# ku222/Attention-GAN

Hardware: AMD Instinct MI355X
Metric: train images/sec at 256×256 stage-3, batch 24/GPU, 1/2/4/8 MI355X (higher is better)
Workload: dtype f32; 1 GPU; full 3-stage AttnGAN 64->128->256 train step: G + 3xD updates + word attention + DAMSM words/sentence loss + KL + 4x fused Adam (BASELINE.json configs[2]); workload_key=full3, batch_per_gpu=24, global_batch=24, gf_dim=32, df_dim=64, emb_dim=256, seq_len=10, text_encoder=bypassed (frozen; N(0,1) embeddings), parallelism=dp1, discriminator_streams=3, launch=eager, gradient_exchange=none (one rank), losses_finite=True

## Files before the change

attention-gan_amd/csrc/conv_wino.hip:

```cpp
#include "conv_common.h"

#include <cstring>

using namespace agan;
using namespace agan::conv;

namespace {

typedef unsigned u32x4 __attribute__((ext_vector_type(4)));

__device__ __forceinline__ void lds_barrier_w() { asm volatile("s_waitcnt lgkmcnt(0)\n\ts_barrier" ::: "memory"); }

__global__ __launch_bounds__(256) void wino_weight_transform_kernel(const float* __restrict__ wk, float* __restrict__ U, int Kin, int Nld, int N) {
    const int total = Kin * Nld;
    for (int e = blockIdx.x * 256 + threadIdx.x; e < total; e += gridDim.x * 256) {
        const int n = e % Nld, c = e / Nld;
        float gk[3][3];
#pragma unroll
        for (int r = 0; r < 3; ++r)
#pragma unroll
            for (int s = 0; s < 3; ++s) gk[r][s] = n < N ? wk[(size_t)(c * 9 + r * 3 + s) * Nld + n] : 0.f;
        float t[4][3];
#pragma unroll
        for (int s = 0; s < 3; ++s) {
            t[0][s] = gk[0][s];
            t[1][s] = 0.5f * (gk[0][s] + gk[1][s] + gk[2][s]);
            t[2][s] = 0.5f * (gk[0][s] - gk[1][s] + gk[2][s]);
            t[3][s] = gk[2][s];
        }
        const int nch8 = Kin >> 3;
#pragma unroll
        for (int xi = 0; xi < 4; ++xi) {
            const float u0 = t[xi][0], u1 = 0.5f * (t[xi][0] + t[xi][1] + t[xi][2]), u2 = 0.5f * (t[xi][0] - t[xi][1] + t[xi][2]), u3 = t[xi][2];
            const float u[4] = {u0, u1, u2, u3};
#pragma unroll
            for (int nu = 0; nu < 4; ++nu) U[((size_t)((xi * 4 + nu) * nch8 + (c >> 3)) * Nld + n) * 8 + (c & 7)] = u[nu];
        }
    }
}

struct WinoTraits {
    int step, extra, origin;
    int cch;
    int planes, classes;
    int stages, nacc;
    int vfrags;
    int pieces;
    int ni32, ni64;
    int lds_cap;
    int s_u_second, s_raw_load, s_u_next, s_transform, s_raw_store;
    bool mulshift;
    bool store1_late;
};
constexpr WinoTraits wino_traits(WinoKind k) {
    WinoTraits t{};
    t.origin = -1; t.classes = 1; t.lds_cap = 160 * 1024; t.s_u_second = 0; t.s_raw_load = 1;
    switch (k) {
    case WinoKind::conv3x3:
        t.step = 2; t.extra = 2; t.cch = 8; t.planes = 16; t.stages = 16; t.nacc = 16; t.vfrags = 16; t.pieces = 4; t.ni32 = 7; t.ni64 = 11;
        t.s_u_next = 8; t.s_transform = 1; t.s_raw_store = 14;
        break;
    case WinoKind::conv3x3_half:
        t.step = 2; t.extra = 2; t.cch = 8; t.planes = 16; t.stages = 8; t.nacc = 8; t.vfrags = 16; t.pieces = 4; t.ni32 = 7;
        t.s_u_next = 4; t.s_transform = 1; t.s_raw_store = 6; t.lds_cap = 80 * 1024; t.mulshift = true;
        break;
    case WinoKind::conv4x4_s2:
        t.step = 4; t.extra = 2; t.cch = 8; t.planes = 36; t.stages = 36; t.nacc = 9; t.vfrags = 36; t.pieces = 4; t.ni32 = 21;
        t.s_u_next = 18; t.s_transform = 2; t.s_raw_store = 32; t.store1_late = true;
        break;
    case WinoKind::dgrad2x2_class:
        t.step = 2; t.extra = 1; t.cch = 16; t.planes = 36; t.classes = 4; t.stages = 18; t.nacc = 9; t.vfrags = 18; t.pieces = 2; t.ni32 = 11;
        t.s_u_next = 9; t.s_transform = 2; t.s_raw_store = 15; t.store1_late = true;
        break;
    }
    return t;
}

template <int D>
__device__ __forceinline__ void wino_input_f22(const float* src, int pcp, float* o, int pp) {
    float t[3][3];
#pragma unroll
    for (int j = 0; j < 3; ++j) {
        const float d0 = src[D * j], d1 = src[D * pcp + D * j], d2 = src[2 * D * pcp + D * j];
        t[0][j] = d0 - d1; t[1][j] = d1; t[2][j] = d2 - d1;
    }
#pragma unroll
    for (int xi = 0; xi < 3; ++xi) {
        o[(xi * 3 + 0) * pp] = t[xi][0] - t[xi][1]; o[(xi * 3 + 1) * pp] = t[xi][1]; o[(xi * 3 + 2) * pp] = t[xi][2] - t[xi][1];
    }
}

template <int NACC>
__device__ __forceinline__ void wino_output_2x2(const f32x16 (&acc)[NACC], int r, float (&y)[4]) {
    if constexpr (NACC == 16) {
        float c0[4], c1[4];
#pragma unroll
        for (int nu = 0; nu < 4; ++nu) {
            c0[nu] = acc[0 + nu][r] + acc[4 + nu][r] + acc[8 + nu][r];
            c1[nu] = acc[4 + nu][r] - acc[8 + nu][r] - acc[12 + nu][r];
        }
        y[0] = c0[0] + c0[1] + c0[2]; y[1] = c0[1] - c0[2] - c0[3];
        y[2] = c1[0] + c1[1] + c1[2]; y[3] = c1[1] - c1[2] - c1[3];
    } else {
        static_assert(NACC == 9, "F(2x2, 3x3) or F(2x2, 2x2)");
        float c0[3], c1[3];
#pragma unroll
        for (int nu = 0; nu < 3; ++nu) {
            c0[nu] = acc[nu][r] + acc[3 + nu][r];
            c1[nu] = acc[3 + nu][r] + acc[6 + nu][r];
        }
        y[0] = c0[0] + c0[1]; y[1] = c0[1] + c0[2];
        y[2] = c1[0] + c1[1]; y[3] = c1[1] + c1[2];
    }
}

template <WinoKind K, int NTG>
struct WinoGather {
    static constexpr WinoTraits T = wino_traits(K);
    static constexpr bool kHalf = K == WinoKind::conv3x3_half, kS2 = K == WinoKind::conv4x4_s2, kCls = K == WinoKind::dgrad2x2_class;
    static constexpr bool k3x3 = T.nacc != 9;
    static constexpr int NFW = kHalf ? 2 : 4 / NTG;
    static constexpr int NTL = 32 * NTG, LT = NTG == 1 ? 5 : 6;
    static constexpr int NI = NTG == 1 ? T.ni32 : T.ni64;
    static constexpr int CCH = T.cch, C8 = T.cch / 8;
    static constexpr int S = T.stages, SH = T.stages / 2, NACC = T.nacc;
    static constexpr int NPIECE = T.pieces * NTG;
    static constexpr int VBUF = T.vfrags * NTL * 8;
    static constexpr int STEP = T.step;
    static_assert(NI > 0, "this block size of the variant is not built: plan_wino must not route to it");
    static_assert(T.s_u_next == SH && T.s_transform + NPIECE <= S && T.s_raw_store < S, "slots of the chunk loop");

    const Geom& g;
    const WinoPlan& wp;
    int tid, lane, w, fw, tg, hh, l31, lh;
    int mt, nt, ks, py, px;
    int n0, txl, tyl, TX, TY, tx0, ty0, tb0, ihw, ohw, PR, PC, PCP, RAWBUF;
    float *raw, *V;
    __amdgpu_buffer_rsrc_t rx, rU;
    int nch8, c_beg, nch;
    int iy0, ix0;

    __device__ __forceinline__ WinoGather(const float* x, const float* U, const Geom& g_, const WinoPlan& wp_) : g(g_), wp(wp_) {
        extern __shared__ __attribute__((aligned(16))) unsigned char lds[];
        tid = threadIdx.x; lane = tid & 63;
        w = __builtin_amdgcn_readfirstlane(tid >> 6);
        fw = w % NFW; tg = kHalf ? 0 : w / NFW; hh = kHalf ? w / NFW : 0;
        l31 = lane & 31; lh = lane >> 5;
        ks = py = px = 0;
        {
            int F = xcd_contiguous(linear_block_id(), wp.mtiles * wp.ntiles * (kS2 ? wp.ksplit : T.classes));
            nt = F % wp.ntiles; F /= wp.ntiles;
            if constexpr (kS2) { mt = F % wp.mtiles; ks = F / wp.mtiles; }
            else if constexpr (kCls) { py = (F & 3) >> 1; px = F & 1; mt = F >> 2; }
            else mt = F;
        }
        n0 = nt * (NFW * 32);
        txl = wp.txl; tyl = wp.tyl;
        TX = 1 << txl; TY = 1 << tyl;
        const int bxi = mt % wp.blocks_x, byi = (mt / wp.blocks_x) % wp.blocks_y, bbi = mt / (wp.blocks_x * wp.blocks_y);
        tx0 = bxi << txl; ty0 = byi << tyl; tb0 = bbi << (LT - txl - tyl);
        ihw = g.IH * g.IW; ohw = g.OH * g.OW;
        PR = STEP * TY + T.extra; PC = STEP * TX + T.extra;
        PCP = wp.pcp;
        raw = reinterpret_cast<float*>(lds);
        RAWBUF = wp.raw_bytes >> 2;
        V = reinterpret_cast<float*>(lds + 2 * wp.raw_bytes);
        nch8 = g.Cin >> 3;
        if constexpr (kS2) { c_beg = ks * wp.chunks_per_split; nch = min(nch8, c_beg + wp.chunks_per_split) - c_beg; }
        else { c_beg = 0; nch = g.Cin >> (CCH == 8 ? 3 : 4); }
        constexpr int PPC = T.planes / T.classes;
        rx = make_rsrc(x, (size_t)g.B * g.Cin * ihw * sizeof(float));
        rU = make_rsrc(U + (size_t)(py * 2 + px) * PPC * nch8 * g.Nld * 8, (size_t)PPC * nch8 * g.Nld * 8 * sizeof(float));
        iy0 = STEP * ty0 + T.origin + py; ix0 = STEP * tx0 + T.origin + px;
    }

    __device__ __forceinline__ void stage_items(int (&it_off)[NI], unsigned (&it_lds)[NI]) const {
#pragma unroll
        for (int i = 0; i < NI; ++i) {
            const int e = tid + i * 256;
            int col, row, t2;
            if constexpr (T.mulshift) {
                const int t1 = (int)(__umul24(e, wp.mpc) >> 16);
                col = e - (int)__umul24(t1, PC);
                t2 = (int)(__umul24(t1, wp.mpr) >> 16); row = t1 - (int)__umul24(t2, PR);
            } else {
                col = e % PC; const int t1 = e / PC;
                row = t1 % PR; t2 = t1 / PR;
            }
            const int ci = t2 & (CCH - 1), b = tb0 + (t2 >> (CCH == 8 ? 3 : 4)), iy = iy0 + row, ix = ix0 + col;
            const bool ok = (e < wp.raw_items) & (b < g.B) & ((unsigned)iy < (unsigned)g.IH) & ((unsigned)ix < (unsigned)g.IW);
            if constexpr (T.mulshift) {
                it_off[i] = ok ? (int)__umul24(b * g.Cin + ci, ihw) + iy * g.IW + ix : -1;
                it_lds[i] = (unsigned)((int)__umul24(__umul24(t2, PR) + row, PCP) + col);
            } else {
                it_off[i] = ok ? (b * g.Cin + ci) * ihw + iy * g.IW + ix : -1;
                it_lds[i] = (unsigned)((t2 * PR + row) * PCP + col);
            }
        }
    }

    __device__ __forceinline__ void load_raw(const int (&it_off)[NI], int ch, float (&rv)[NI]) const {
#pragma unroll
        for (int i = 0; i < NI; ++i)
            rv[i] = buf_load_s(rx, it_off[i] >= 0 ? (unsigned)it_off[i] * 4u : kOOB, (unsigned)((c_beg + ch) * CCH * ihw) * 4u);
    }
    __device__ __forceinline__ void store_raw(const unsigned (&it_lds)[NI], int ch, const float (&rv)[NI]) const {
        float* const rb = raw + (ch & 1) * RAWBUF;
#pragma unroll
        for (int i = 0; i < NI; ++i)
            if (tid + i * 256 < wp.raw_items) rb[it_lds[i]] = rv[i];
    }
    __device__ __forceinline__ void load_u(int ch, int half, u32x4 (&uf)[SH]) const {
        const unsigned ulane = (unsigned)(min(n0 + fw * 32 + l31, g.Nld - 1) * 32 + lh * 16);
#pragma unroll
        for (int q = 0; q < SH; ++q) {
            const int s = half * SH + q;
            uf[q] = __builtin_bit_cast(u32x4, __builtin_amdgcn_raw_buffer_load_b128(
                rU, ulane, (unsigned)(((hh * S + s / C8) * nch8 + (c_beg + min(ch, nch - 1)) * C8 + s % C8) * g.Nld) * 32u, 0));
        }
    }

    __device__ __forceinline__ void transform_piece(const float* rb, float* Vb, int pi, float (&td)[NTG][4][4]) const {
        const int k = pi / T.pieces, sub = pi % T.pieces;
        const int tt = (tid >> 3) + 32 * k, ci = (tid & 7) + (kCls ? 8 * sub : 0);
        const int p = kS2 ? sub >> 1 : 0, q = kS2 ? sub & 1 : 0;
        if (!k3x3 || sub == 0) {
            const int ttx = tt & (TX - 1), tty = (tt >> txl) & (TY - 1), ttb = tt >> (txl + tyl);
            const float* const src = rb + ((ttb * CCH + ci) * PR + STEP * tty + p) * PCP + STEP * ttx + q;
            if constexpr (k3x3) {
                float d[4][4];
#pragma unroll
                for (int i = 0; i < 4; ++i) {
                    const float2 a = *reinterpret_cast<const float2*>(src + i * PCP), b = *reinterpret_cast<const float2*>(src + i * PCP + 2);
                    d[i][0] = a.x; d[i][1] = a.y; d[i][2] = b.x; d[i][3] = b.y;
                }
#pragma unroll
                for (int j = 0; j < 4; ++j) {
                    td[k][0][j] = d[0][j] - d[2][j];
                    td[k][1][j] = d[1][j] + d[2][j];
                    td[k][2][j] = d[2][j] - d[1][j];
                    td[k][3][j] = d[1][j] - d[3][j];
                }
            } else if constexpr (kS2) wino_input_f22<2>(src, PCP, Vb + (sub * 9 * NTL + tt) * 8 + ci, NTL * 8);
            else wino_input_f22<1>(src, PCP, Vb + tt * 16 + ci, NTL * 16);
        }
        if constexpr (k3x3) {
            const float (&t)[4] = td[k][sub];
            float* const o = Vb + (sub * 4 * NTL + tt) * 8 + ci;
            o[0] = t[0] - t[2]; o[NTL * 8] = t[1] + t[2]; o[2 * NTL * 8] = t[2] - t[1]; o[3 * NTL * 8] = t[1] - t[3];
        }
    }

    __device__ __forceinline__ void accumulate(f32x16 (&acc)[NACC]) const {
        int it_off[NI];
        unsigned it_lds[NI];
        stage_items(it_off, it_lds);
        float rawv[NI];
        float td[NTG][4][4];
        u32x4 ua[SH], ub[SH];
#pragma unroll
        for (int q = 0; q < NACC; ++q)
#pragma unroll
            for (int r = 0; r < 16; ++r) acc[q][r] = 0.f;
        {
            float rawv1[NI];
            load_raw(it_off, 0, rawv);
            if (!T.store1_late && nch > 1) load_raw(it_off, 1, rawv1);
            load_u(0, 0, ua);
            store_raw(it_lds, 0, rawv);
            if (nch > 1) {
                if constexpr (T.store1_late) load_raw(it_off, 1, rawv);
                else store_raw(it_lds, 1, rawv1);
            }
            lds_barrier_w();
#pragma unroll
            for (int pi = 0; pi < NPIECE; ++pi) transform_piece(raw, V, pi, td);
            if (T.store1_late && nch > 1) store_raw(it_lds, 1, rawv);
            lds_barrier_w();
        }
#pragma unroll 1
        for (int ch = 0; ch < nch; ++ch) {
            const float* Vc = V + (ch & 1) * VBUF;
            float* Vn = V + ((ch + 1) & 1) * VBUF;
            const float* rn = raw + ((ch + 1) & 1) * RAWBUF;
            const bool more = ch + 1 < nch;
            const unsigned vlane = (unsigned)(hh * S * NTL * 8 + (tg * 32 + l31) * CCH + lh * 4);
            u32x4 vf[2];
            vf[0] = *reinterpret_cast<const u32x4*>(Vc + vlane);
#pragma unroll
            for (int st = 0; st < S; ++st) {
                if (st + 1 < S) vf[(st + 1) & 1] = *reinterpret_cast<const u32x4*>(Vc + ((st + 1) / C8) * NTL * CCH + ((st + 1) % C8) * 8 + vlane);
                if (st == T.s_u_second) load_u(ch, 1, ub);
                if (st == T.s_raw_load && ch + 2 < nch) load_raw(it_off, ch + 2, rawv);
                if (st == T.s_u_next) load_u(ch + 1, 0, ua);
                if (more && st >= T.s_transform && st < T.s_transform + NPIECE) transform_piece(rn, Vn, st - T.s_transform, td);
                if (st == T.s_raw_store && ch + 2 < nch) store_raw(it_lds, ch + 2, rawv);
                const u32x4 uf = st < SH ? ua[st % SH] : ub[st % SH];
                const int a = kS2 ? st % NACC : st / C8;
#pragma unroll
                for (int j = 0; j < 4; ++j)
                    acc[a] = __builtin_amdgcn_mfma_f32_32x32x2f32(__uint_as_float(uf[j]), __uint_as_float(vf[st & 1][j]), acc[a], 0, 0, 0);
                __builtin_amdgcn_sched_barrier(0);
            }
            lds_barrier_w();
        }
    }

    __device__ __forceinline__ void epilogue(const f32x16 (&acc)[NACC], float* out) const {
        typedef float f32x2_ __attribute__((ext_vector_type(2)));
        typedef unsigned u32x2_ __attribute__((ext_vector_type(2)));
        const int lt = tg * 32 + l31;
        const int tx = lt & (TX - 1), ty = (lt >> txl) & (TY - 1), tb = lt >> (txl + tyl);
        const int b = tb0 + tb, oy = 2 * (ty0 + ty), ox = 2 * (tx0 + tx);
        const bool pvalid = (b < g.B) & (oy < (kCls ? g.OHs : g.OH)) & (ox < (kCls ? g.OWs : g.OW));
        const __amdgpu_buffer_rsrc_t ro = make_rsrc(out + (size_t)ks * wp.slab, (size_t)g.B * g.Cout * ohw * sizeof(float));
        const int nw = n0 + fw * 32;
#pragma unroll
        for (int r = 0; r < 16; ++r) {
            float y[4];
            wino_output_2x2(acc, r, y);
            const int n = nw + (r & 3) + 8 * (r >> 2) + 4 * lh;
            const bool ok = pvalid & (n < g.Cout);
            if constexpr (kCls) {
                const unsigned off = (unsigned)((b * g.Cout + n) * ohw + (2 * oy + py) * g.OW + 2 * ox + px) * 4u;
                buf_store(ro, ok ? off : kOOB, y[0]);
                buf_store(ro, ok ? off + 8u : kOOB, y[1]);
                buf_store(ro, ok ? off + (unsigned)(2 * g.OW) * 4u : kOOB, y[2]);
                buf_store(ro, ok ? off + (unsigned)(2 * g.OW + 2) * 4u : kOOB, y[3]);
            } else {
                const unsigned off = (unsigned)((b * g.Cout + n) * ohw + oy * g.OW + ox) * 4u;
                __builtin_amdgcn_raw_buffer_store_b64(__builtin_bit_cast(u32x2_, f32x2_{y[0], y[1]}), ro, ok ? off : kOOB, 0, 0);
                __builtin_amdgcn_raw_buffer_store_b64(__builtin_bit_cast(u32x2_, f32x2_{y[2], y[3]}), ro, ok ? off + (unsigned)g.OW * 4u : kOOB, 0, 0);
            }
        }
    }
};

template <int NFW>
__global__ __launch_bounds__(256, 1) void conv_wino_f32_kernel(const float* __restrict__ x, const float* __restrict__ U, float* __restrict__ out,
                                                               const Geom g, const WinoPlan wp) {
    WinoGather<WinoKind::conv3x3, 4 / NFW> k(x, U, g, wp);
    f32x16 acc[k.NACC];
    k.accumulate(acc);
    k.epilogue(acc, out);
}

__global__ __launch_bounds__(256, 2) void conv_wino_h_f32_kernel(const float* __restrict__ x, const float* __restrict__ U, float* __restrict__ out,
                                                                 const Geom g, const WinoPlan wp) {
    WinoGather<WinoKind::conv3x3_half, 1> k(x, U, g, wp);
    f32x16 acc[8];
    k.accumulate(acc);

    const int w = k.w, lane = k.lane, hh = k.hh, ohw = k.ohw;
    float* const X = k.raw;
    typedef float f32x2_ __attribute__((ext_vector_type(2)));
    typedef unsigned u32x2_ __attribute__((ext_vector_type(2)));
    const int tx = k.l31 & (k.TX - 1), ty = (k.l31 >> k.txl) & (k.TY - 1), tb = k.l31 >> (k.txl + k.tyl);
    const int b = k.tb0 + tb, oy = 2 * (k.ty0 + ty) + hh, ox = 2 * (k.tx0 + tx);
    const bool pvalid = (b < g.B) & (oy < g.OH) & (ox < g.OW);
    const __amdgpu_buffer_rsrc_t ro = make_rsrc(out, (size_t)g.B * g.Cout * ohw * sizeof(float));
    const int nw = k.n0 + k.fw * 32, pw = w ^ 2;
    const unsigned vo = pvalid ? (unsigned)((b * g.Cout + nw + 4 * k.lh) * ohw + oy * g.OW + ox) * 4u : kOOB;
    auto finish = [&](auto hc) {
        constexpr int HH = decltype(hc)::value;
        f32x2_ keep[8][2];
#pragma unroll
        for (int rp = 0; rp < 8; ++rp) {
            f32x2_ t[2][2];
#pragma unroll
            for (int x2 = 0; x2 < 2; ++x2) {
                const f32x2_ m0 = {acc[x2 * 4 + 0][2 * rp], acc[x2 * 4 + 0][2 * rp + 1]};
                const f32x2_ m1 = {acc[x2 * 4 + 1][2 * rp], acc[x2 * 4 + 1][2 * rp + 1]};
                const f32x2_ m2 = {acc[x2 * 4 + 2][2 * rp], acc[x2 * 4 + 2][2 * rp + 1]};
                const f32x2_ m3 = {acc[x2 * 4 + 3][2 * rp], acc[x2 * 4 + 3][2 * rp + 1]};
                t[x2][0] = m0 + m1 + m2;
                t[x2][1] = m1 - m2 - m3;
            }
#pragma unroll
            for (int c = 0; c < 2; ++c) {
                keep[rp][c] = t[0][c] + t[1][c];
                const f32x2_ send = HH == 0 ? t[1][c] : t[0][c];
                X[(w * 32 + (2 * rp) * 2 + c) * 64 + lane] = send[0];
                X[(w * 32 + (2 * rp + 1) * 2 + c) * 64 + lane] = send[1];
            }
        }
        lds_barrier_w();
#pragma unroll
        for (int r = 0; r < 16; ++r) {
            if (nw + 8 * (r >> 2) < g.Cout) {
                const float x0 = X[(pw * 32 + r * 2 + 0) * 64 + lane], x1 = X[(pw * 32 + r * 2 + 1) * 64 + lane];
                const float k0 = keep[r >> 1][0][r & 1], k1 = keep[r >> 1][1][r & 1];
                const f32x2_ y = HH == 0 ? f32x2_{x0 + k0, x1 + k1} : f32x2_{x0 - k0, x1 - k1};
                __builtin_amdgcn_raw_buffer_store_b64(__builtin_bit_cast(u32x2_, y), ro, vo, (unsigned)(((r & 3) + 8 * (r >> 2)) * ohw) * 4u, 0);
            }
        }
    };
    if (hh == 0) finish(std::integral_constant<int, 0>{});
    else finish(std::integral_constant<int, 1>{});
}

template <int NFW>
__global__ __launch_bounds__(256, 1) void conv_wino_s2_f32_kernel(const float* __restrict__ x, const float* __restrict__ U, float* __restrict__ out,
                                                                  const Geom g, const WinoPlan wp) {
    WinoGather<WinoKind::conv4x4_s2, 4 / NFW> k(x, U, g, wp);
    f32x16 acc[k.NACC];
    k.accumulate(acc);
    k.epilogue(acc, out);
}

template <int NFW>
__global__ __launch_bounds__(256, 1) void conv_wino_cls_f32_kernel(const float* __restrict__ x, const float* __restrict__ U, float* __restrict__ out,
                                                                   const Geom g, const WinoPlan wp) {
    WinoGather<WinoKind::dgrad2x2_class, 4 / NFW> k(x, U, g, wp);
    f32x16 acc[k.NACC];
    k.accumulate(acc);
    k.epilogue(acc, out);
}

__device__ __forceinline__ void wino_weights_f22(const float (&gk)[2][2], float* o, size_t pp) {
    const float t[3][2] = {{gk[0][0], gk[0][1]}, {gk[0][0] + gk[1][0], gk[0][1] + gk[1][1]}, {gk[1][0], gk[1][1]}};
#pragma unroll
    for (int xi = 0; xi < 3; ++xi) {
        const float u[3] = {t[xi][0], t[xi][0] + t[xi][1], t[xi][1]};
#pragma unroll
        for (int nu = 0; nu < 3; ++nu) o[(xi * 3 + nu) * pp] = u[nu];
    }
}

__global__ __launch_bounds__(256) void wino_cls_weight_transform_kernel(const float* __restrict__ wk, float* __restrict__ U, int Kin, int Nld, int N) {
    const int total = 4 * Kin * Nld, nch8 = Kin >> 3;
    for (int e = blockIdx.x * 256 + threadIdx.x; e < total; e += gridDim.x * 256) {
        const int n = e % Nld, t1 = e / Nld, c = t1 % Kin, cls = t1 / Kin;
        const float* wc = wk + (size_t)cls * Kin * 4 * Nld;
        float gk[2][2];
#pragma unroll
        for (int a = 0; a < 2; ++a)
#pragma unroll
            for (int b = 0; b < 2; ++b) gk[a][b] = n < N ? wc[(size_t)(c * 4 + (1 - a) * 2 + (1 - b)) * Nld + n] : 0.f;
        wino_weights_f22(gk, U + ((size_t)(cls * 9 * nch8 + (c >> 3)) * Nld + n) * 8 + (c & 7), (size_t)nch8 * Nld * 8);
    }
}

__global__ __launch_bounds__(256) void wino_s2_weight_transform_kernel(const float* __restrict__ wk, float* __restrict__ U, int Kin, int Nld, int N) {
    const int total = Kin * Nld, nch8 = Kin >> 3;
    for (int e = blockIdx.x * 256 + threadIdx.x; e < total; e += gridDim.x * 256) {
        const int n = e % Nld, c = e / Nld;
#pragma unroll
        for (int p = 0; p < 2; ++p)
#pragma unroll
            for (int q = 0; q < 2; ++q) {
                float gk[2][2];
#pragma unroll
                for (int a = 0; a < 2; ++a)
#pragma unroll
                    for (int b = 0; b < 2; ++b) gk[a][b] = n < N ? wk[(size_t)(c * 16 + (2 * a + p) * 4 + 2 * b + q) * Nld + n] : 0.f;
                wino_weights_f22(gk, U + ((size_t)((p * 2 + q) * 9 * nch8 + (c >> 3)) * Nld + n) * 8 + (c & 7), (size_t)nch8 * Nld * 8);
            }
    }
}

__global__ __launch_bounds__(256, 1) void conv_wino_wgrad_f32_kernel(const float* __restrict__ x, const float* __restrict__ dy, float* __restrict__ part,
                                                                     const Geom g, const WinoWgradPlan wp) {
    extern __shared__ __attribute__((aligned(16))) unsigned char lds[];
    constexpr int ZV = 16 * 64 * 8;
    float* const L = reinterpret_cast<float*>(lds);
    const int tid = threadIdx.x, lane = tid & 63;
    const int w = __builtin_amdgcn_readfirstlane(tid >> 6);
    const int fj = w & 1, fi = w >> 1;
    const int l31 = lane & 31, lh = lane >> 5;
    int jt, it, split;
    {
        int F = xcd_contiguous(linear_block_id(), wp.jtiles * wp.itiles * wp.psplit);
        jt = F % wp.jtiles; F /= wp.jtiles;
        it = F % wp.itiles; split = F / wp.itiles;
    }
    const int j0 = jt * 64, i0 = it * 64;
    const int ihw = g.IH * g.IW;
    const int o_beg = split * wp.octs_per_split, o_end = min(wp.noct, o_beg + wp.octs_per_split);
    const __amdgpu_buffer_rsrc_t rx = make_rsrc(x, (size_t)g.B * g.Cin * ihw * sizeof(float));
    const __amdgpu_buffer_rsrc_t rd = make_rsrc(dy, (size_t)g.B * g.Cout * ihw * sizeof(float));
    const int tw8 = g.OW >> 4, th = g.OH >> 1;

    const int tj = tid & 7, tc = tid >> 3;
    float xr[2][16];
    float2 dr[2][2];
    auto load_piece = [&](int o, int lp) {
        const bool ov = o < o_end;
        const int txo = o % tw8, t1 = o / tw8;
        const int ty = t1 % th, b = t1 / th;
        const int tx = txo * 8 + tj;
        const int k = lp >> 1, half = lp & 1;
        const int ci = i0 + tc + 32 * k, co = j0 + tc + 32 * k;
        const bool cv = ov & (ci < g.Cin);
        const int xbase = (b * g.Cin + ci) * ihw + 2 * tx - 1;
        const bool c0ok = tx > 0, c3ok = 2 * tx + 2 < g.IW;
#pragma unroll
        for (int ii = 0; ii < 2; ++ii) {
            const int i = 2 * half + ii;
            const int iy = 2 * ty - 1 + i;
            const bool rv = cv & ((unsigned)iy < (unsigned)g.IH);
            const unsigned ro = (unsigned)(xbase + iy * g.IW) * 4u;
            xr[k][i * 4 + 0] = buf_load(rx, (rv & c0ok) ? ro : kOOB);
            xr[k][i * 4 + 1] = buf_load(rx, rv ? ro + 4u : kOOB);
            xr[k][i * 4 + 2] = buf_load(rx, rv ? ro + 8u : kOOB);
            xr[k][i * 4 + 3] = buf_load(rx, (rv & c3ok) ? ro + 12u : kOOB);
        }
        if (half == 0) {
            const bool dv = ov & (co < g.Cout);
            const int dbase = (b * g.Cout + co) * ihw + 2 * ty * g.OW + 2 * tx;
#pragma unroll
            for (int a = 0; a < 2; ++a)
                dr[k][a] = __builtin_bit_cast(float2, __builtin_amdgcn_raw_buffer_load_b64(rd, dv ? (unsigned)(dbase + a * g.OW) * 4u : kOOB, 0, 0));
        }
    };
    auto load_oct = [&](int o) {
#pragma unroll
        for (int lp = 0; lp < 4; ++lp) load_piece(o, lp);
    };
    float tt_[2][4][4];
    auto transform_piece = [&](float* buf, int tp) {
        const int k = tp >> 2, sub = tp & 3;
        const int ch = tc + 32 * k;
        if (sub == 0) {
#pragma unroll
            for (int c = 0; c < 4; ++c) {
                const float d0 = xr[k][c], d1 = xr[k][4 + c], d2 = xr[k][8 + c], d3 = xr[k][12 + c];
                tt_[k][0][c] = d0 - d2; tt_[k][1][c] = d1 + d2; tt_[k][2][c] = d2 - d1; tt_[k][3][c] = d3 - d1;
            }
        }
        if (sub < 2) {
#pragma unroll
            for (int x2 = 0; x2 < 2; ++x2) {
                const int xi = 2 * sub + x2;
                const float* t = tt_[k][xi];
                float* o = buf + ZV + ((xi * 4) * 64 + ch) * 8 + tj;
                o[0] = t[0] - t[2]; o[64 * 8] = t[1] + t[2]; o[2 * 64 * 8] = t[2] - t[1]; o[3 * 64 * 8] = t[3] - t[1];
            }
        } else {
            const float e00 = dr[k][0].x, e01 = dr[k][0].y, e10 = dr[k][1].x, e11 = dr[k][1].y;
#pragma unroll
            for (int x2 = 0; x2 < 2; ++x2) {
                const int xi = 2 * (sub - 2) + x2;
                const float u0 = xi == 0 ? e00 : (xi == 1 ? 0.5f * (e00 + e10) : (xi == 2 ? 0.5f * (e00 - e10) : e10));
                const float u1 = xi == 0 ? e01 : (xi == 1 ? 0.5f * (e01 + e11) : (xi == 2 ? 0.5f * (e01 - e11) : e11));
                float* o = buf + ((xi * 4) * 64 + ch) * 8 + tj;
                o[0] = u0; o[64 * 8] = 0.5f * (u0 + u1); o[2 * 64 * 8] = 0.5f * (u0 - u1); o[3 * 64 * 8] = u1;
            }
        }
    };
    auto transform_store = [&](float* buf) {
#pragma unroll
        for (int tp = 0; tp < 8; ++tp) transform_piece(buf, tp);
    };

    f32x16 acc[16];
#pragma unroll
    for (int q = 0; q < 16; ++q)
#pragma unroll
        for (int r = 0; r < 16; ++r) acc[q][r] = 0.f;

    if (o_beg < o_end) {
        load_oct(o_beg);
        transform_store(L);
        load_oct(o_beg + 1);
        lds_barrier_w();
        const unsigned zl = (unsigned)((fj * 32 + l31) * 8 + lh * 4), vl = (unsigned)(ZV + (fi * 32 + l31) * 8 + lh * 4);
        for (int o = o_beg; o < o_end; ++o) {
            const float* cur = L + ((o - o_beg) & 1) * (2 * ZV);
            float* nxt = L + (((o - o_beg) & 1) ^ 1) * (2 * ZV);
            u32x4 zf[2], vf[2];
            zf[0] = *reinterpret_cast<const u32x4*>(cur + zl);
            vf[0] = *reinterpret_cast<const u32x4*>(cur + vl);
#pragma unroll
            for (int pos = 0; pos < 16; ++pos) {
                if (pos + 1 < 16) {
                    zf[(pos + 1) & 1] = *reinterpret_cast<const u32x4*>(cur + (pos + 1) * 64 * 8 + zl);
                    vf[(pos + 1) & 1] = *reinterpret_cast<const u32x4*>(cur + (pos + 1) * 64 * 8 + vl);
                }
                if (pos >= 1 && pos <= 8) transform_piece(nxt, pos - 1);
                if (pos >= 9 && pos <= 12) load_piece(o + 2, pos - 9);
#pragma unroll
                for (int j = 0; j < 4; ++j)
                    acc[pos] = __builtin_amdgcn_mfma_f32_32x32x2f32(__uint_as_float(zf[pos & 1][j]), __uint_as_float(vf[pos & 1][j]), acc[pos], 0, 0, 0);
#pragma unroll
                for (int j = 0; j < 4; ++j) {
                    __builtin_amdgcn_sched_group_barrier(0x008, 1, 0);
                    __builtin_amdgcn_sched_group_barrier(0x100, 1, 0);
                    __builtin_amdgcn_sched_group_barrier(0x002, 8, 0);
                    __builtin_amdgcn_sched_group_barrier(0x020, 3, 0);
                    __builtin_amdgcn_sched_group_barrier(0x200, 1, 0);
                }
                __builtin_amdgcn_sched_barrier(0);
            }
            lds_barrier_w();
        }
    }

    float* const o = part + (size_t)split * wp.slab;
    const __amdgpu_buffer_rsrc_t ro = make_rsrc(o, (size_t)9 * g.Cout * g.Cin * sizeof(float));
    const int ci = i0 + fi * 32 + l31;
    const int cob = j0 + fj * 32;
    const unsigned vo = ci < g.Cin ? (unsigned)(4 * lh * g.Cin + ci) * 4u : kOOB;
    const unsigned tapb = (unsigned)(g.Cout * g.Cin) * 4u;
#pragma unroll
    for (int r = 0; r < 16; ++r) {
        if (cob + 8 * (r >> 2) >= g.Cout) continue;
        float c[3][4];
#pragma unroll
        for (int nu = 0; nu < 4; ++nu) {
            const float m0 = acc[nu][r], m1 = acc[4 + nu][r], m2 = acc[8 + nu][r], m3 = acc[12 + nu][r];
            c[0][nu] = m0 + m1 + m2;
            c[1][nu] = m1 - m2;
            c[2][nu] = m1 + m2 + m3;
        }
        const unsigned so = (unsigned)((cob + (r & 3) + 8 * (r >> 2)) * g.Cin) * 4u;
#pragma unroll
        for (int rr = 0; rr < 3; ++rr) {
            __builtin_amdgcn_raw_buffer_store_b32(__builtin_bit_cast(unsigned, c[rr][0] + c[rr][1] + c[rr][2]), ro, vo, so + (unsigned)(rr * 3 + 0) * tapb, 0);
            __builtin_amdgcn_raw_buffer_store_b32(__builtin_bit_cast(unsigned, c[rr][1] - c[rr][2]), ro, vo, so + (unsigned)(rr * 3 + 1) * tapb, 0);
            __builtin_amdgcn_raw_buffer_store_b32(__builtin_bit_cast(unsigned, c[rr][1] + c[rr][2] + c[rr][3]), ro, vo, so + (unsigned)(rr * 3 + 2) * tapb, 0);
        }
    }
}

__global__ __launch_bounds__(256) void wino_wgrad_sum_kernel(const float* __restrict__ part, int nslabs, size_t slab, int cout, int cin,
                                                             float* __restrict__ dw, int accumulate) {
    __shared__ f32x4 red[8][32];
    const int q4 = cin >> 2, n4 = 9 * cout * q4;
    const int el = threadIdx.x & 31, grp = threadIdx.x >> 5;
    for (int base = blockIdx.x * 32; base < n4; base += gridDim.x * 32) {
        const int e = base + el;
        f32x4 a = {0.f, 0.f, 0.f, 0.f};
        if (e < n4) {
            const float* src = part + (size_t)e * 4;
            int sp = grp;
            for (; sp + 24 < nslabs; sp += 32) {
                const f32x4 v0 = *reinterpret_cast<const f32x4*>(src + (size_t)sp * slab);
                const f32x4 v1 = *reinterpret_cast<const f32x4*>(src + (size_t)(sp + 8) * slab);
                const f32x4 v2 = *reinterpret_cast<const f32x4*>(src + (size_t)(sp + 16) * slab);
                const f32x4 v3 = *reinterpret_cast<const f32x4*>(src + (size_t)(sp + 24) * slab);
                a += (v0 + v1) + (v2 + v3);
            }
            for (; sp < nslabs; sp += 8) a += *reinterpret_cast<const f32x4*>(src + (size_t)sp * slab);
        }
        red[grp][el] = a;
        __syncthreads();
        if (grp == 0 && e < n4) {
#pragma unroll
            for (int k = 1; k < 8; ++k) a += red[k][el];
            const int c4 = e % q4, t1 = e / q4;
            const int co = t1 % cout, tap = t1 / cout;
            float* dst = dw + ((size_t)co * cin + 4 * c4) * 9 + tap;
#pragma unroll
            for (int k = 0; k < 4; ++k) dst[k * 9] = accumulate ? dst[k * 9] + a[k] : a[k];
        }
        __syncthreads();
    }
}

int pow2floor_log(int v) {
    int l = 0;
    while ((2 << l) <= v) ++l;
    return l;
}

}

namespace agan {
namespace conv {

WinoPlan plan_wino(const Geom& g) {
    WinoPlan p;
    memset(&p, 0, sizeof(p));
    if (g.SY == 1 && g.R == 3 && g.S == 3 && g.DY == 1 && g.OS == 1 && g.OY0 == -1 && g.IH == g.OH && g.IW == g.OW)
        p.kind = (g.Cout & 7) == 0 ? WinoKind::conv3x3_half : WinoKind::conv3x3;
    else if (g.SY == 2 && g.R == 4 && g.S == 4 && g.DY == 1 && g.OS == 1 && g.OY0 == -1 && g.IH == 2 * g.OH && g.IW == 2 * g.OW) p.kind = WinoKind::conv4x4_s2;
    else if (g.SY == 1 && g.R == 2 && g.S == 2 && g.DY == -1 && g.OS == 2 && g.OY0 == 0 && g.OY1 == 1 && g.OH == 2 * g.IH && g.OW == 2 * g.IW) p.kind = WinoKind::dgrad2x2_class;
    else return p;
    const WinoTraits T = wino_traits(p.kind);
    const bool k3x3 = p.kind == WinoKind::conv3x3 || p.kind == WinoKind::conv3x3_half;
    if ((g.OHs & 1) || (g.OWs & 1) || (g.Cin & (T.cch - 1)) || g.Cout < 32) return p;
    if (!k3x3 && g.Cout < 96) return p;
    const int tw = g.OWs / 2, th = g.OHs / 2;
    if (tw < 4) return p;
    p.nf = (g.Cout >= 96 || p.kind == WinoKind::conv3x3_half) ? 4 : 2;
    const int lt = p.nf == 4 ? 5 : 6;
    p.txl = std::min(3, pow2floor_log(tw));
    p.tyl = std::min(lt - p.txl, pow2floor_log(th));
    const int TX = 1 << p.txl, TY = 1 << p.tyl, TB = (1 << lt) >> (p.txl + p.tyl);
    p.blocks_x = cdiv(tw, TX);
    p.blocks_y = cdiv(th, TY);
    p.blocks_b = cdiv(g.B, TB);
    p.mtiles = p.blocks_x * p.blocks_y * p.blocks_b;
    p.ntiles = p.kind == WinoKind::conv3x3_half ? cdiv(g.Cout, 64) : cdiv(g.Cout, p.nf * 32);
    p.ksplit = 1;
    if (p.kind == WinoKind::conv4x4_s2 && p.mtiles * p.ntiles < 512 && p.mtiles * p.ntiles >= 256 && g.Cin >= 128) p.ksplit = 2;
    if (p.mtiles * p.ntiles * p.ksplit * T.classes < (k3x3 ? 256 : 512)) return p;
    p.chunks_per_split = cdiv(g.Cin / 8, p.ksplit);
    p.slab = ((size_t)g.B * g.Cout * g.OH * g.OW + 3) / 4 * 4;
    const int PR = T.step * TY + T.extra, PC = T.step * TX + T.extra;
    p.pcp = (PC + 1) & ~1;
    p.mpc = (65536 + PC - 1) / PC;
    p.mpr = (65536 + PR - 1) / PR;
    p.raw_items = TB * T.cch * PR * PC;
    if (p.raw_items > (lt == 5 ? T.ni32 : T.ni64) * 256) return p;
    p.raw_bytes = (TB * T.cch * PR * p.pcp * 4 + 15) & ~15;
    p.smem_bytes = 2 * p.raw_bytes + 2 * T.vfrags * (1 << lt) * 8 * 4;
    if (p.smem_bytes > T.lds_cap) return p;
    p.u_bytes = ((size_t)T.planes * (g.Cin / 8) * g.Nld * 8 * sizeof(float) + 255) / 256 * 256;
    p.ws_bytes = p.u_bytes + (p.ksplit > 1 ? p.slab * p.ksplit * sizeof(float) : 0);
    p.ok = 1;
    return p;
}

namespace {
template <auto Kernel, WinoKind K>
void launch_gather_kernel(dim3 grid, const float* in, const float* U, float* out, const Geom& g, const WinoPlan& p, hipStream_t st) {
    allow_dynamic_lds<Kernel>(wino_traits(K).lds_cap);
    AGAN_LAUNCH(Kernel, grid, dim3(256), (size_t)p.smem_bytes, st, in, U, out, g, p);
}
}

void launch_wino(const float* in, const float* wk, float* out, const Geom& g, const WinoPlan& p, void* ws, hipStream_t st) {
    float* U = static_cast<float*>(ws);
    const int total = g.Cin * g.Nld;
    const dim3 grid(p.mtiles * p.ntiles * p.ksplit * wino_traits(p.kind).classes), tgrid(std::min(cdiv(total, 256), 2048));
    switch (p.kind) {
    case WinoKind::dgrad2x2_class:
        AGAN_LAUNCH(wino_cls_weight_transform_kernel, dim3(std::min(cdiv(4 * total, 256), 4096)), dim3(256), 0, st, wk, U, g.Cin, g.Nld, g.Cout);
        launch_gather_kernel<conv_wino_cls_f32_kernel<4>, WinoKind::dgrad2x2_class>(grid, in, U, out, g, p, st);
        break;
    case WinoKind::conv4x4_s2:
        AGAN_LAUNCH(wino_s2_weight_transform_kernel, tgrid, dim3(256), 0, st, wk, U, g.Cin, g.Nld, g.Cout);
        launch_gather_kernel<conv_wino_s2_f32_kernel<4>, WinoKind::conv4x4_s2>(
            grid, in, U, p.ksplit > 1 ? reinterpret_cast<float*>(static_cast<char*>(ws) + p.u_bytes) : out, g, p, st);
        break;
    case WinoKind::conv3x3_half:
        AGAN_LAUNCH(wino_weight_transform_kernel, tgrid, dim3(256), 0, st, wk, U, g.Cin, g.Nld, g.Cout);
        launch_gather_kernel<conv_wino_h_f32_kernel, WinoKind::conv3x3_half>(grid, in, U, out, g, p, st);
        break;
    case WinoKind::conv3x3:
        AGAN_LAUNCH(wino_weight_transform_kernel, tgrid, dim3(256), 0, st, wk, U, g.Cin, g.Nld, g.Cout);
        if (p.nf == 4) launch_gather_kernel<conv_wino_f32_kernel<4>, WinoKind::conv3x3>(grid, in, U, out, g, p, st);
        else launch_gather_kernel<conv_wino_f32_kernel<2>, WinoKind::conv3x3>(grid, in, U, out, g, p, st);
        break;
    }
}

WinoWgradPlan plan_wino_wgrad(const Geom& g) {
    WinoWgradPlan p;
    memset(&p, 0, sizeof(p));
    if (!(g.SY == 1 && g.R == 3 && g.S == 3 && g.DY == 1 && g.OS == 1 && g.OY0 == -1)) return p;
    if (g.IH != g.OH || g.IW != g.OW || (g.OH & 1) || (g.OW & 15) || g.Cin < 32 || g.Cout < 32 || (g.Cin & 3) || (g.Cout & 7)) return p;
    p.noct = g.B * (g.OH / 2) * (g.OW / 16);
    p.jtiles = cdiv(g.Cout, 64);
    p.itiles = cdiv(g.Cin, 64);
    const int wgs = p.jtiles * p.itiles;
    if (p.noct < 64 * 16 || wgs > 256) return p;
    const int ps = std::max(1, std::min(256 / wgs, p.noct / 16));
    p.octs_per_split = cdiv(p.noct, ps);
    p.psplit = cdiv(p.noct, p.octs_per_split);
    p.slab = ((size_t)g.Cout * g.Cin * 9 + 3) / 4 * 4;
    p.ws_bytes = p.slab * p.psplit * sizeof(float);
    p.smem_bytes = 2 * 2 * 16 * 64 * 8 * 4;
    p.ok = 1;
    return p;
}

void launch_wino_wgrad(const float* x, const float* dy, float* part, const Geom& g, const WinoWgradPlan& p, hipStream_t st) {
    allow_dynamic_lds<conv_wino_wgrad_f32_kernel>(160 * 1024);
    AGAN_LAUNCH(conv_wino_wgrad_f32_kernel, dim3(p.jtiles * p.itiles * p.psplit), dim3(256), (size_t)p.smem_bytes, st, x, dy, part, g, p);
}

void launch_wino_wgrad_sum(const float* part, const Geom& g, const WinoWgradPlan& p, float* dw, int accumulate, hipStream_t st) {
    const int n4 = 9 * g.Cout * (g.Cin >> 2);
    AGAN_LAUNCH(wino_wgrad_sum_kernel, dim3(std::min(cdiv(n4, 32), 8192)), dim3(256), 0, st, part, p.psplit, p.slab, g.Cout, g.Cin, dw, accumulate);
}

}
}
```

profiles/conv_micro.py:

```python
import argparse
import importlib
import os
import sys

import torch

ROOT = os.path.dirname(os.path.dirname(os.path.abspath(__file__)))
sys.path.insert(0, ROOT)
HF = importlib.import_module("attention-gan_amd.backend.functional")
L = importlib.import_module("attention-gan_amd.backend.lib")

LAYERS = {
    "d_down_64_128": ("down", 48, 64, 128, 128, 4),
    "d_down_128_256": ("down", 48, 128, 64, 256, 4),
    "d_down_256_512": ("down", 48, 256, 32, 512, 4),
    "d_down_512_1024": ("down", 48, 512, 16, 1024, 4),
    "d_down_1024_2048": ("down", 48, 1024, 8, 2048, 4),
    "g_same_64_128": ("same", 24, 64, 128, 128, 3),
    "g_same_64_64": ("same", 24, 64, 128, 64, 3),
    "g_up_64_64": ("up", 24, 64, 128, 64, 3),
    "syn_same_256_128": ("same", 24, 256, 64, 128, 3),
    "rgb_head_256": ("same", 24, 32, 256, 3, 3),
    "rgb_head_128": ("same", 24, 32, 128, 3, 3),
}


def main():
    ap = argparse.ArgumentParser()
    ap.add_argument("--precision", default="bf16")
    ap.add_argument("--storage", default="f32")
    ap.add_argument("--layers", default="all")
    ap.add_argument("--iters", type=int, default=20)
    ap.add_argument("--phases", default="fwd,dgrad,wgrad")
    a = ap.parse_args()
    HF.set_precision(L.PRECISIONS[a.precision])
    HF.set_activation_storage(None if a.storage == "f32" else a.storage)
    tdt = {"f32": torch.float32, "bf16": torch.bfloat16, "f16": torch.float16}[a.storage]
    names = list(LAYERS) if a.layers == "all" else [n for n in LAYERS if any(n.startswith(p) for p in a.layers.split(","))]
    dev = "cuda"
    print(f"{'layer':18s} {'phase':6s} {'us':>8s} {'TF/s':>8s} {'GB/s':>8s}")
    for name in names:
        kind, B, Cin, H, Cout, k = LAYERS[name]
        g = torch.Generator().manual_seed(1)
        x = torch.randn(B, Cin, H, H, generator=g).to(dev).to(tdt)
        w = (torch.randn(Cout, Cin, k, k, generator=g) / (Cin * k * k) ** 0.5).to(dev)
        cache = {}
        OH = H // 2 if kind == "down" else (2 * H if kind == "up" else H)
        flops = 2.0 * B * OH * OH * Cout * Cin * (k * k if kind != "up" else 9)
        esz = x.element_size()
        nbytes = esz * (x.numel() + B * Cout * OH * OH)
        for phase in a.phases.split(","):
            xr = x.clone().requires_grad_(phase == "dgrad")
            wr = w.clone().requires_grad_(phase == "wgrad")
            y = HF.conv2d(xr, wr, None, kind, cache)
            gy = torch.randn(y.shape, generator=torch.Generator(device=dev).manual_seed(2), device=dev).to(y.dtype)

            def run():
                if phase == "fwd":
                    HF.conv2d(xr, wr, None, kind, cache)
                else:
                    torch.autograd.grad(y, xr if phase == "dgrad" else wr, gy, retain_graph=True)
            for _ in range(3):
                run()
            best = 1e9
            for _ in range(3):
                e0, e1 = torch.cuda.Event(enable_timing=True), torch.cuda.Event(enable_timing=True)
                torch.cuda.synchronize()
                e0.record()
                for _ in range(a.iters):
                    run()
                e1.record()
                torch.cuda.synchronize()
                best = min(best, e0.elapsed_time(e1) / a.iters * 1e3)
            print(f"{name:18s} {phase:6s} {best:8.1f} {flops / best / 1e6:8.1f} {nbytes / best / 1e3:8.1f}", flush=True)


if __name__ == "__main__":
    main()
```

Before: 1002 images/s.

## Split Winograd wgrad into two half-tile blocks for higher occupancy

Splits the F(2,3) Winograd weight-gradient kernel into two halves, each covering 8 of the 16 transform positions. This halves the accumulators and LDS per block, so launch bounds can allow 2 blocks per CU, and the grid and partial-sum workspace double. Input loading now uses per-row buffer resources and b64 loads, with DPP lane shuffles supplying neighbouring columns, and the output transform is rewritten per half with a sign factor. The split heuristic also changes. The costs are extra workspace and a larger final reduction, plus more complex edge handling that could be wrong at borders.

Result: no change. 1009 images/s (median of 6 runs) (+0.8%).

```diff
diff --git a/attention-gan_amd/csrc/conv_wino.hip b/attention-gan_amd/csrc/conv_wino.hip
--- a/attention-gan_amd/csrc/conv_wino.hip
+++ b/attention-gan_amd/csrc/conv_wino.hip
@@ -459,103 +459,123 @@
     }
 }
 
-__global__ __launch_bounds__(256, 1) void conv_wino_wgrad_f32_kernel(const float* __restrict__ x, const float* __restrict__ dy, float* __restrict__ part,
+constexpr int kWgradHalves = 2;
+__global__ __launch_bounds__(256, 2) void conv_wino_wgrad_f32_kernel(const float* __restrict__ x, const float* __restrict__ dy, float* __restrict__ part,
                                                                      const Geom g, const WinoWgradPlan wp) {
     extern __shared__ __attribute__((aligned(16))) unsigned char lds[];
-    constexpr int ZV = 16 * 64 * 8;
+    constexpr int NP = 16 / kWgradHalves;
+    constexpr int ZV = NP * 64 * 8;
     float* const L = reinterpret_cast<float*>(lds);
     const int tid = threadIdx.x, lane = tid & 63;
     const int w = __builtin_amdgcn_readfirstlane(tid >> 6);
     const int fj = w & 1, fi = w >> 1;
     const int l31 = lane & 31, lh = lane >> 5;
-    int jt, it, split;
+    int jt, it, split, h;
     {
-        int F = xcd_contiguous(linear_block_id(), wp.jtiles * wp.itiles * wp.psplit);
+        int F = xcd_contiguous(linear_block_id(), kWgradHalves * wp.jtiles * wp.itiles * wp.psplit);
+        h = F & 1; F >>= 1;
         jt = F % wp.jtiles; F /= wp.jtiles;
         it = F % wp.itiles; split = F / wp.itiles;
     }
+    const float sgn = h ? -1.f : 1.f;
     const int j0 = jt * 64, i0 = it * 64;
     const int ihw = g.IH * g.IW;
     const int o_beg = split * wp.octs_per_split, o_end = min(wp.noct, o_beg + wp.octs_per_split);
-    const __amdgpu_buffer_rsrc_t rx = make_rsrc(x, (size_t)g.B * g.Cin * ihw * sizeof(float));
-    const __amdgpu_buffer_rsrc_t rd = make_rsrc(dy, (size_t)g.B * g.Cout * ihw * sizeof(float));
     const int tw8 = g.OW >> 4, th = g.OH >> 1;
 
     const int tj = tid & 7, tc = tid >> 3;
-    float xr[2][16];
+    float xr[2][12];
     float2 dr[2][2];
+    constexpr unsigned kFar = 0xFFFFFF00u;
+    unsigned vx[2], ve[2], vd[2];
+#pragma unroll
+    for (int k = 0; k < 2; ++k) {
+        const unsigned vo = (unsigned)((tc + 32 * k) * ihw + 2 * tj) * 4u;
+        const bool xv = i0 + tc + 32 * k < g.Cin;
+        vx[k] = xv ? vo : kFar;
+        ve[k] = !xv ? kFar : (tj == 0 ? vo : (tj == 7 ? vo + 12u : kFar));
+        vd[k] = j0 + tc + 32 * k < g.Cout ? vo : kFar;
+    }
+    const size_t xbytes = (size_t)g.B * g.Cin * ihw * sizeof(float), dbytes = (size_t)g.B * g.Cout * ihw * sizeof(float);
     auto load_piece = [&](int o, int lp) {
         const bool ov = o < o_end;
         const int txo = o % tw8, t1 = o / tw8;
         const int ty = t1 % th, b = t1 / th;
-        const int tx = txo * 8 + tj;
-        const int k = lp >> 1, half = lp & 1;
-        const int ci = i0 + tc + 32 * k, co = j0 + tc + 32 * k;
-        const bool cv = ov & (ci < g.Cin);
-        const int xbase = (b * g.Cin + ci) * ihw + 2 * tx - 1;
-        const bool c0ok = tx > 0, c3ok = 2 * tx + 2 < g.IW;
-#pragma unroll
-        for (int ii = 0; ii < 2; ++ii) {
-            const int i = 2 * half + ii;
+        const int k = lp >> 1;
+        auto row_rsrc = [&](const float* t, size_t bytes, long long first, bool valid) {
+            const long long skip = valid ? first * 4 : 0;
+            return make_rsrc(reinterpret_cast<const char*>(t) + skip, valid ? bytes - (size_t)skip : 0);
+        };
+        auto load_row = [&](int slot, int i) {
             const int iy = 2 * ty - 1 + i;
-            const bool rv = cv & ((unsigned)iy < (unsigned)g.IH);
-            const unsigned ro = (unsigned)(xbase + iy * g.IW) * 4u;
-            xr[k][i * 4 + 0] = buf_load(rx, (rv & c0ok) ? ro : kOOB);
-            xr[k][i * 4 + 1] = buf_load(rx, rv ? ro + 4u : kOOB);
-            xr[k][i * 4 + 2] = buf_load(rx, rv ? ro + 8u : kOOB);
-            xr[k][i * 4 + 3] = buf_load(rx, (rv & c3ok) ? ro + 12u : kOOB);
-        }
-        if (half == 0) {
-            const bool dv = ov & (co < g.Cout);
-            const int dbase = (b * g.Cout + co) * ihw + 2 * ty * g.OW + 2 * tx;
-#pragma unroll
-            for (int a = 0; a < 2; ++a)
-                dr[k][a] = __builtin_bit_cast(float2, __builtin_amdgcn_raw_buffer_load_b64(rd, dv ? (unsigned)(dbase + a * g.OW) * 4u : kOOB, 0, 0));
+            const __amdgpu_buffer_rsrc_t r =
+                row_rsrc(x, xbytes, (long long)(b * g.Cin + i0) * ihw + iy * g.IW + 16 * txo - 1, ov & ((unsigned)iy < (unsigned)g.IH));
+            const float2 m = __builtin_bit_cast(float2, __builtin_amdgcn_raw_buffer_load_b64(r, vx[k], 4u, 0));
+            xr[k][slot * 4 + 1] = m.x;
+            xr[k][slot * 4 + 2] = m.y;
+            const bool edge = ((txo == 0) & (tj == 0)) | ((txo == tw8 - 1) & (tj == 7));
+            xr[k][slot * 4 + 0] = buf_load_s(r, edge ? kFar : ve[k], 0u);
+        };
+        if ((lp & 1) == 0) {
+            load_row(0, 3 * h);
+            load_row(1, 1 + h);
+        } else {
+            load_row(2, 2 - h);
+#pragma unroll
+            for (int a = 0; a < 2; ++a) {
+                const __amdgpu_buffer_rsrc_t r = row_rsrc(dy, dbytes, (long long)(b * g.Cout + j0) * ihw + (2 * ty + (a ^ h)) * g.OW + 16 * txo, ov);
+                dr[k][a] = __builtin_bit_cast(float2, __builtin_amdgcn_raw_buffer_load_b64(r, vd[k], 0, 0));
+            }
         }
     };
     auto load_oct = [&](int o) {
 #pragma unroll
         for (int lp = 0; lp < 4; ++lp) load_piece(o, lp);
     };
-    float tt_[2][4][4];
     auto transform_piece = [&](float* buf, int tp) {
-        const int k = tp >> 2, sub = tp & 3;
-        const int ch = tc + 32 * k;
-        if (sub == 0) {
+        const int k = tp >> 1;
+        float* o = buf + (tc + 32 * k) * 8 + tj;
+        if ((tp & 1) == 0) {
+            float d[3][4];
+#pragma unroll
+            for (int row = 0; row < 3; ++row) {
+                const int e = __builtin_bit_cast(int, xr[k][row * 4]);
+                const int left = __builtin_amdgcn_update_dpp(0, __builtin_bit_cast(int, xr[k][row * 4 + 2]), 0x111, 0xf, 0xf, true);
+                const int right = __builtin_amdgcn_update_dpp(0, __builtin_bit_cast(int, xr[k][row * 4 + 1]), 0x101, 0xf, 0xf, true);
+                d[row][0] = __builtin_bit_cast(float, tj == 0 ? e : left);
+                d[row][1] = xr[k][row * 4 + 1];
+                d[row][2] = xr[k][row * 4 + 2];
+                d[row][3] = __builtin_bit_cast(float, tj == 7 ? e : right);
+            }
+            float t[2][4];
 #pragma unroll
             for (int c = 0; c < 4; ++c) {
-                const float d0 = xr[k][c], d1 = xr[k][4 + c], d2 = xr[k][8 + c], d3 = xr[k][12 + c];
-                tt_[k][0][c] = d0 - d2; tt_[k][1][c] = d1 + d2; tt_[k][2][c] = d2 - d1; tt_[k][3][c] = d3 - d1;
-            }
-        }
-        if (sub < 2) {
-#pragma unroll
-            for (int x2 = 0; x2 < 2; ++x2) {
-                const int xi = 2 * sub + x2;
-                const float* t = tt_[k][xi];
-                float* o = buf + ZV + ((xi * 4) * 64 + ch) * 8 + tj;
-                o[0] = t[0] - t[2]; o[64 * 8] = t[1] + t[2]; o[2 * 64 * 8] = t[2] - t[1]; o[3 * 64 * 8] = t[3] - t[1];
+                t[0][c] = d[0][c] - d[2][c];
+                t[1][c] = __builtin_fmaf(d[2][c], sgn, d[1][c]);
+            }
+#pragma unroll
+            for (int lr = 0; lr < 2; ++lr) {
+                float* ov = o + ZV + lr * 4 * 64 * 8;
+                ov[0] = t[lr][0] - t[lr][2]; ov[64 * 8] = t[lr][1] + t[lr][2]; ov[2 * 64 * 8] = t[lr][2] - t[lr][1]; ov[3 * 64 * 8] = t[lr][3] - t[lr][1];
             }
         } else {
-            const float e00 = dr[k][0].x, e01 = dr[k][0].y, e10 = dr[k][1].x, e11 = dr[k][1].y;
-#pragma unroll
-            for (int x2 = 0; x2 < 2; ++x2) {
-                const int xi = 2 * (sub - 2) + x2;
-                const float u0 = xi == 0 ? e00 : (xi == 1 ? 0.5f * (e00 + e10) : (xi == 2 ? 0.5f * (e00 - e10) : e10));
-                const float u1 = xi == 0 ? e01 : (xi == 1 ? 0.5f * (e01 + e11) : (xi == 2 ? 0.5f * (e01 - e11) : e11));
-                float* o = buf + ((xi * 4) * 64 + ch) * 8 + tj;
-                o[0] = u0; o[64 * 8] = 0.5f * (u0 + u1); o[2 * 64 * 8] = 0.5f * (u0 - u1); o[3 * 64 * 8] = u1;
+            const float u[2][2] = {{dr[k][0].x, dr[k][0].y},
+                                   {0.5f * __builtin_fmaf(dr[k][0].x, sgn, dr[k][1].x), 0.5f * __builtin_fmaf(dr[k][0].y, sgn, dr[k][1].y)}};
+#pragma unroll
+            for (int lr = 0; lr < 2; ++lr) {
+                float* oz = o + lr * 4 * 64 * 8;
+                oz[0] = u[lr][0]; oz[64 * 8] = 0.5f * (u[lr][0] + u[lr][1]); oz[2 * 64 * 8] = 0.5f * (u[lr][0] - u[lr][1]); oz[3 * 64 * 8] = u[lr][1];
             }
         }
     };
     auto transform_store = [&](float* buf) {
 #pragma unroll
-        for (int tp = 0; tp < 8; ++tp) transform_piece(buf, tp);
+        for (int tp = 0; tp < 4; ++tp) transform_piece(buf, tp);
     };
 
-    f32x16 acc[16];
-#pragma unroll
-    for (int q = 0; q < 16; ++q)
+    f32x16 acc[NP];
+#pragma unroll
+    for (int q = 0; q < NP; ++q)
 #pragma unroll
         for (int r = 0; r < 16; ++r) acc[q][r] = 0.f;
 
@@ -572,13 +592,13 @@
             zf[0] = *reinterpret_cast<const u32x4*>(cur + zl);
             vf[0] = *reinterpret_cast<const u32x4*>(cur + vl);
 #pragma unroll
-            for (int pos = 0; pos < 16; ++pos) {
-                if (pos + 1 < 16) {
+            for (int pos = 0; pos < NP; ++pos) {
+                if (pos + 1 < NP) {
                     zf[(pos + 1) & 1] = *reinterpret_cast<const u32x4*>(cur + (pos + 1) * 64 * 8 + zl);
                     vf[(pos + 1) & 1] = *reinterpret_cast<const u32x4*>(cur + (pos + 1) * 64 * 8 + vl);
                 }
-                if (pos >= 1 && pos <= 8) transform_piece(nxt, pos - 1);
-                if (pos >= 9 && pos <= 12) load_piece(o + 2, pos - 9);
+                if ((pos & 3) < 2) transform_piece(nxt, 2 * (pos >> 2) + (pos & 1));
+                else load_piece(o + 2, 2 * (pos >> 2) + (pos & 1));
 #pragma unroll
                 for (int j = 0; j < 4; ++j)
                     acc[pos] = __builtin_amdgcn_mfma_f32_32x32x2f32(__uint_as_float(zf[pos & 1][j]), __uint_as_float(vf[pos & 1][j]), acc[pos], 0, 0, 0);
@@ -588,7 +608,7 @@
                     __builtin_amdgcn_sched_group_barrier(0x100, 1, 0);
                     __builtin_amdgcn_sched_group_barrier(0x002, 8, 0);
                     __builtin_amdgcn_sched_group_barrier(0x020, 3, 0);
-                    __builtin_amdgcn_sched_group_barrier(0x200, 1, 0);
+                    __builtin_amdgcn_sched_group_barrier(0x200, 2, 0);
                 }
                 __builtin_amdgcn_sched_barrier(0);
             }
@@ -596,7 +616,7 @@
         }
     }
 
-    float* const o = part + (size_t)split * wp.slab;
+    float* const o = part + (size_t)(split * kWgradHalves + h) * wp.slab;
     const __amdgpu_buffer_rsrc_t ro = make_rsrc(o, (size_t)9 * g.Cout * g.Cin * sizeof(float));
     const int ci = i0 + fi * 32 + l31;
     const int cob = j0 + fj * 32;
@@ -608,10 +628,10 @@
         float c[3][4];
 #pragma unroll
         for (int nu = 0; nu < 4; ++nu) {
-            const float m0 = acc[nu][r], m1 = acc[4 + nu][r], m2 = acc[8 + nu][r], m3 = acc[12 + nu][r];
-            c[0][nu] = m0 + m1 + m2;
-            c[1][nu] = m1 - m2;
-            c[2][nu] = m1 + m2 + m3;
+            const float mb = acc[4 + nu][r], s = acc[nu][r] + mb;
+            c[0][nu] = h ? mb : s;
+            c[1][nu] = h ? -mb : mb;
+            c[2][nu] = h ? s : mb;
         }
         const unsigned so = (unsigned)((cob + (r & 3) + 8 * (r >> 2)) * g.Cin) * 4u;
 #pragma unroll
@@ -757,25 +777,26 @@
     p.itiles = cdiv(g.Cin, 64);
     const int wgs = p.jtiles * p.itiles;
     if (p.noct < 64 * 16 || wgs > 256) return p;
-    const int ps = std::max(1, std::min(256 / wgs, p.noct / 16));
+    const int ps = std::max(1, std::min(256 / wgs, p.noct / 12));
     p.octs_per_split = cdiv(p.noct, ps);
     p.psplit = cdiv(p.noct, p.octs_per_split);
     p.slab = ((size_t)g.Cout * g.Cin * 9 + 3) / 4 * 4;
-    p.ws_bytes = p.slab * p.psplit * sizeof(float);
-    p.smem_bytes = 2 * 2 * 16 * 64 * 8 * 4;
+    p.ws_bytes = p.slab * p.psplit * kWgradHalves * sizeof(float);
+    p.smem_bytes = 2 * 2 * (16 / kWgradHalves) * 64 * 8 * 4;
     p.ok = 1;
     return p;
 }
 
 void launch_wino_wgrad(const float* x, const float* dy, float* part, const Geom& g, const WinoWgradPlan& p, hipStream_t st) {
-    allow_dynamic_lds<conv_wino_wgrad_f32_kernel>(160 * 1024);
-    AGAN_LAUNCH(conv_wino_wgrad_f32_kernel, dim3(p.jtiles * p.itiles * p.psplit), dim3(256), (size_t)p.smem_bytes, st, x, dy, part, g, p);
+    allow_dynamic_lds<conv_wino_wgrad_f32_kernel>(80 * 1024);
+    AGAN_LAUNCH(conv_wino_wgrad_f32_kernel, dim3(p.jtiles * p.itiles * p.psplit * kWgradHalves), dim3(256), (size_t)p.smem_bytes, st, x, dy, part, g, p);
 }
 
 void launch_wino_wgrad_sum(const float* part, const Geom& g, const WinoWgradPlan& p, float* dw, int accumulate, hipStream_t st) {
     const int n4 = 9 * g.Cout * (g.Cin >> 2);
-    AGAN_LAUNCH(wino_wgrad_sum_kernel, dim3(std::min(cdiv(n4, 32), 8192)), dim3(256), 0, st, part, p.psplit, p.slab, g.Cout, g.Cin, dw, accumulate);
-}
-
-}
-}
+    AGAN_LAUNCH(wino_wgrad_sum_kernel, dim3(std::min(cdiv(n4, 32), 8192)), dim3(256), 0, st, part, p.psplit * kWgradHalves, p.slab, g.Cout, g.Cin, dw,
+                accumulate);
+}
+
+}
+}
diff --git a/profiles/conv_micro.py b/profiles/conv_micro.py
--- a/profiles/conv_micro.py
+++ b/profiles/conv_micro.py
@@ -18,7 +18,9 @@
     "d_down_1024_2048": ("down", 48, 1024, 8, 2048, 4),
     "g_same_64_128": ("same", 24, 64, 128, 128, 3),
     "g_same_64_64": ("same", 24, 64, 128, 64, 3),
-    "g_up_64_64": ("up", 24, 64, 128, 64, 3),
+    "g_same_h64_64_128": ("same", 24, 64, 64, 128, 3),
+    "g_same_h64_64_64": ("same", 24, 64, 64, 64, 3),
+    "g_up_64_64":("up", 24, 64, 128, 64, 3),
     "syn_same_256_128": ("same", 24, 256, 64, 128, 3),
     "rgb_head_256": ("same", 24, 32, 256, 3, 3),
     "rgb_head_128": ("same", 24, 32, 128, 3, 3),
```
